# LRMPUT/PUTSLAM

Hardware: AMD Instinct MI355X
Metric: frame-pairs/s (match+RANSAC+Kabsch), 640x480 @ 2000 kpts (higher is better)
Workload: dtype f32; 1 GPU; BASELINE configs[2]: TUM fr1/desk-style synthetic sequence, 500 frames = 499 frame pairs per step per GPU, 2000 kpts/frame, 256-bit descriptors, Hamming BF + cross-check -> depth filter -> H=4096 3-pt Umeyama hypotheses (fixed) scored with errorVersion 1 -> refit; inputs resident in HBM; kpts=2000, hypotheses=4096, world_size=1, force_dist=False, estimator=fixed, streams=4, join=end, submit=ps_batch_queue_submit: whole batches to the library's chains in turn, matcher_kernel=mfma-fused, score_kernel=fast, hw_queues=4, accepted_pairs=499

## Files before the change

putslam_amd/csrc/ps_matcher_mfma.h:

```cpp
#pragma once

#include "ps_kernels.h"

namespace psdev {

typedef int v4i_t __attribute__((ext_vector_type(4)));
typedef int v8i_t __attribute__((ext_vector_type(8)));
typedef float v16f_t __attribute__((ext_vector_type(16)));

constexpr int kTileRows = 32;
constexpr int kTileU4 = 256;
constexpr int kWavesPerWG = kBlock / 64;

PS_D uint32_t fp4_from_byte(uint32_t x)
{
    x = (x | (x << 12)) & 0x000F000Fu;
    x = (x | (x << 6)) & 0x03030303u;
    x = (x | (x << 3)) & 0x11111111u;
    return (x << 3) | 0x66666666u;
}
PS_D v4i_t fp4_from_dword(uint32_t w)
{
    v4i_t r;
    r.x = (int)fp4_from_byte(w & 0xFFu);
    r.y = (int)fp4_from_byte((w >> 8) & 0xFFu);
    r.z = (int)fp4_from_byte((w >> 16) & 0xFFu);
    r.w = (int)fp4_from_byte(w >> 24);
    return r;
}

PS_D int tile_row(int reg, int h) { return (reg & 3) + 8 * (reg >> 2) + 4 * h; }

__global__ __launch_bounds__(kBlock) void ps_expand_query_fp4(const uint32_t *__restrict__ desc,
                                                              const int32_t *__restrict__ nkpts,
                                                              const int32_t *__restrict__ pairs, int cap, int fstride, int tpf,
                                                              int chunks, uint4 *__restrict__ Xq,
                                                              uint32_t *__restrict__ keysInit)
{
    const int p = (int)(blockIdx.x / (unsigned)chunks), chunk = (int)(blockIdx.x % (unsigned)chunks);
    if (keysInit)
        for (int t = chunk * kBlock + threadIdx.x; t < cap; t += chunks * kBlock) keysInit[(size_t)p * cap + t] = kNoKey;
    const int fq = pairs[2 * p];
    const int nq = nkpts[fq];
    const uint32_t *__restrict__ q32 = desc + (size_t)fq * fstride;
    uint4 *__restrict__ out = Xq + (size_t)p * tpf * kTileU4;
    const int o = threadIdx.x, s = o >> 6, h = (o >> 5) & 1, r = o & 31;
    for (int tile = chunk; tile < tpf; tile += chunks) {
        const int row = tile * kTileRows + r;
        v4i_t e = {0, 0, 0, 0};
        if (row < nq) e = fp4_from_dword(q32[(size_t)row * 8 + 2 * s + h]);
        out[(size_t)tile * kTileU4 + o] = make_uint4((uint32_t)e.x, (uint32_t)e.y, (uint32_t)e.z, (uint32_t)e.w);
    }
}

PS_D v16f_t mfma_fp4(const v4i_t &a, const v4i_t &b, const v16f_t &c)
{
    const v8i_t a8 = __builtin_shufflevector(a, a, 0, 1, 2, 3, -1, -1, -1, -1);
    const v8i_t b8 = __builtin_shufflevector(b, b, 0, 1, 2, 3, -1, -1, -1, -1);
    return __builtin_amdgcn_mfma_scale_f32_32x32x64_f8f6f4(a8, b8, c, 4, 4, 0, 0, 0, 0);
}

PS_D v16f_t mfma_fp4s(const v4i_t &a, const v4i_t &b, const v16f_t &c)
{
    const v8i_t a8 = __builtin_shufflevector(a, a, 0, 1, 2, 3, -1, -1, -1, -1);
    const v8i_t b8 = __builtin_shufflevector(b, b, 0, 1, 2, 3, -1, -1, -1, -1);
    return __builtin_amdgcn_mfma_scale_f32_32x32x64_f8f6f4(a8, b8, c, 4, 4, 0, (int)0x88888888u, 0, (int)0x7F7F7F7Fu);
}

PS_D int fbits(float f) { return __builtin_bit_cast(int, f); }
PS_D int imax3(int a, int b, int c) { return max(max(a, b), c); }
PS_D int max16(const v16f_t &d)
{
    int m = imax3(fbits(d[0]), fbits(d[1]), fbits(d[2]));
    m = imax3(m, fbits(d[3]), fbits(d[4]));
    m = imax3(m, fbits(d[5]), fbits(d[6]));
    m = imax3(m, fbits(d[7]), fbits(d[8]));
    m = imax3(m, fbits(d[9]), fbits(d[10]));
    m = imax3(m, fbits(d[11]), fbits(d[12]));
    m = imax3(m, fbits(d[13]), fbits(d[14]));
    return max(m, fbits(d[15]));
}

constexpr float kMfmaNoRow = -1.0e30f;
constexpr int kMfmaBias = 8223;
constexpr float kMfmaBase = 8388608.0f;

#ifndef PS_MFMA_WAVES
#define PS_MFMA_WAVES 1
#endif
template <int TT>
__global__ __launch_bounds__(kBlock, PS_MFMA_WAVES) void ps_hamming_mfma(const uint32_t *__restrict__ desc,
                                                          const int32_t *__restrict__ nkpts,
                                                          const int32_t *__restrict__ pairs, int cap, int fstride, int tpf,
                                                          int groups, int qsplit, const uint4 *__restrict__ Xq,
                                                          uint32_t *__restrict__ keys)
{
    const unsigned perPair = (unsigned)(groups * qsplit);
    const unsigned L = xcd_remap(blockIdx.x, gridDim.x);
    const int p = (int)(L / perPair);
    const int inner = (int)(L - (unsigned)p * perPair);
    const int g = inner / qsplit, qs = inner - g * qsplit;
    const int fq = pairs[2 * p], ft = pairs[2 * p + 1];
    const int nq = nkpts[fq], nt = nkpts[ft];
    if (g * (kWavesPerWG * TT * kTileRows) >= nt) return;
    const int tid = threadIdx.x, lane = tid & 63, wave = tid >> 6;
    const int r = lane & 31, h = lane >> 5;
    const int tile0 = (g * kWavesPerWG + wave) * TT;
    const int nqTiles = (nq + kTileRows - 1) / kTileRows;
    const int T0 = (int)(((long long)nqTiles * qs) / qsplit), T1 = (int)(((long long)nqTiles * (qs + 1)) / qsplit);

    const uint32_t *__restrict__ t32 = desc + (size_t)ft * fstride;
    v4i_t B[TT][4];
#pragma unroll
    for (int i = 0; i < TT; ++i) {
        int t = (tile0 + i) * kTileRows + r;
        t = t < nt ? t : nt - 1;
#pragma unroll
        for (int s = 0; s < 4; ++s) B[i][s] = fp4_from_dword(t32[(size_t)t * 8 + 2 * s + h]);
    }
    v16f_t C;
#pragma unroll
    for (int reg = 0; reg < 16; ++reg) C[reg] = kMfmaBase + (float)(kMfmaBias - 4096 - tile_row(reg, h));
    int best[TT], bestT[TT];
#pragma unroll
    for (int i = 0; i < TT; ++i) {
        best[i] = 0;
        bestT[i] = 0;
    }

    const uint4 *__restrict__ xq = Xq + (size_t)p * tpf * kTileU4;
    uint4 an[4];
    if (T0 < T1) {
#pragma unroll
        for (int s = 0; s < 4; ++s) an[s] = xq[(size_t)T0 * kTileU4 + s * 64 + lane];
    }
    for (int T = T0; T < T1; ++T) {
        v4i_t A[4];
#pragma unroll
        for (int s = 0; s < 4; ++s) {
            A[s].x = (int)an[s].x; A[s].y = (int)an[s].y; A[s].z = (int)an[s].z; A[s].w = (int)an[s].w;
        }
        if (T + 1 < T1) {
#pragma unroll
            for (int s = 0; s < 4; ++s) an[s] = xq[(size_t)(T + 1) * kTileU4 + s * 64 + lane];
        }
        v16f_t Cin = C;
        if (T * kTileRows + kTileRows > nq) {
#pragma unroll
            for (int reg = 0; reg < 16; ++reg)
                if (T * kTileRows + tile_row(reg, h) >= nq) Cin[reg] = kMfmaNoRow;
        }
#pragma unroll
        for (int i = 0; i < TT; ++i) {
            v16f_t acc = mfma_fp4(A[0], B[i][0], Cin);
            acc = mfma_fp4(A[1], B[i][1], acc);
            acc = mfma_fp4(A[2], B[i][2], acc);
            acc = mfma_fp4(A[3], B[i][3], acc);
            const int m = max16(acc);
            if (m > (best[i] | 31)) {
                best[i] = m;
                bestT[i] = T;
            }
        }
    }
#pragma unroll
    for (int i = 0; i < TT; ++i) {
        const int t = (tile0 + i) * kTileRows + r;
        uint32_t key = kNoKey;
        if (best[i] > 0) {
            const int v = kMfmaBias - (best[i] & 0x7FFFFF);
            key = ((uint32_t)(v >> 5) << 16) | (uint32_t)(bestT[i] * kTileRows + (v & 31));
        }
        const uint32_t other = (uint32_t)__shfl_xor((int)key, 32, 64);
        key = other < key ? other : key;
        if (h == 0 && t < nt) {
            if (qsplit == 1)
                keys[(size_t)p * cap + t] = key;
            else
                atomicMin(&keys[(size_t)p * cap + t], key);
        }
    }
}

constexpr int kFuseChunk = 4;

template <int TT>
__global__ __launch_bounds__(kBlock, PS_MFMA_WAVES) void ps_hamming_mfma_fused(const uint32_t *__restrict__ desc,
                                                                const int32_t *__restrict__ nkpts,
                                                                const int32_t *__restrict__ pairs, int cap, int fstride, int tpf,
                                                                int groups, int qsplit, uint32_t *__restrict__ keys)
{
    __shared__ uint4 s_a[2][kFuseChunk][kTileU4];
    __shared__ uint32_t s_lut[256];
    s_lut[threadIdx.x] = fp4_from_byte(threadIdx.x);
    const unsigned perPair = (unsigned)(groups * qsplit);
    const unsigned L = xcd_remap(blockIdx.x, gridDim.x);
    const int p = (int)(L / perPair);
    const int inner = (int)(L - (unsigned)p * perPair);
    const int g = inner / qsplit, qs = inner - g * qsplit;
    const int fq = pairs[2 * p], ft = pairs[2 * p + 1];
    const int nq = nkpts[fq], nt = nkpts[ft];
    if (g * (kWavesPerWG * TT * kTileRows) >= nt) return;
    const int tid = threadIdx.x, lane = tid & 63, wave = tid >> 6;
    const int r = lane & 31, h = lane >> 5;
    const int tile0 = (g * kWavesPerWG + wave) * TT;
    const int nqTiles = (nq + kTileRows - 1) / kTileRows;
    const int T0 = (int)(((long long)nqTiles * qs) / qsplit), T1 = (int)(((long long)nqTiles * (qs + 1)) / qsplit);

    const uint32_t *__restrict__ t32 = desc + (size_t)ft * fstride;
    v4i_t B[TT][4];
#pragma unroll
    for (int i = 0; i < TT; ++i) {
        int t = (tile0 + i) * kTileRows + r;
        t = t < nt ? t : nt - 1;
#pragma unroll
        for (int s = 0; s < 4; ++s) B[i][s] = fp4_from_dword(t32[(size_t)t * 8 + 2 * s + h]);
    }
    v16f_t C;
#pragma unroll
    for (int reg = 0; reg < 16; ++reg) C[reg] = kMfmaBase + (float)((1 << 21) + 31 - tile_row(reg, h));
    int best[TT];
#pragma unroll
    for (int i = 0; i < TT; ++i) best[i] = 0;

    const uint32_t *__restrict__ q32 = desc + (size_t)fq * fstride;
    const int es = tid >> 6, eh = (tid >> 5) & 1, er = tid & 31;
    const int lastT = (nq & (kTileRows - 1)) ? nqTiles - 1 : -1;
    const bool hasPartial = lastT >= T0 && lastT < T1;
    const int Tm = hasPartial ? lastT : T1;
    auto expand_tile = [&](uint4 *dst, int T) {
        const int row = T * kTileRows + er;
        v4i_t e = {0, 0, 0, 0};
        if (row < nq) {
            const uint32_t w = q32[(size_t)row * 8 + 2 * es + eh];
            e.x = (int)s_lut[w & 0xFFu];
            e.y = (int)s_lut[(w >> 8) & 0xFFu];
            e.z = (int)s_lut[(w >> 16) & 0xFFu];
            e.w = (int)s_lut[w >> 24];
        }
        dst[tid] = make_uint4((uint32_t)e.x, (uint32_t)e.y, (uint32_t)e.z, (uint32_t)e.w);
    };
    auto expand_chunk = [&](int buf, int Tc) {
#pragma unroll
        for (int j = 0; j < kFuseChunk; ++j)
            if (Tc + j < Tm) expand_tile(s_a[buf][j], Tc + j);
    };
    auto tile_body = [&](int T, const uint4 *__restrict__ tile, const v16f_t &Cin) {
        v4i_t A[4];
#pragma unroll
        for (int s = 0; s < 4; ++s) {
            const uint4 a = tile[s * 64 + lane];
            A[s].x = (int)a.x; A[s].y = (int)a.y; A[s].z = (int)a.z; A[s].w = (int)a.w;
        }
        const int cT = 16352 - 32 * T;
#pragma unroll
        for (int i = 0; i < TT; ++i) {
            v16f_t acc = mfma_fp4s(A[0], B[i][0], Cin);
            acc = mfma_fp4s(A[1], B[i][1], acc);
            acc = mfma_fp4s(A[2], B[i][2], acc);
            acc = mfma_fp4s(A[3], B[i][3], acc);
            best[i] = max(best[i], max16(acc) + cT);
        }
    };
    __syncthreads();
    if (T0 < Tm) expand_chunk(0, T0);
    __syncthreads();
    int c = 0;
    for (int Tc = T0; Tc < Tm; Tc += kFuseChunk, ++c) {
        if (Tc + kFuseChunk < Tm) expand_chunk((c + 1) & 1, Tc + kFuseChunk);
#pragma unroll 1
        for (int j = 0; j < kFuseChunk; ++j) {
            if (Tc + j >= Tm) break;
            tile_body(Tc + j, s_a[c & 1][j], C);
        }
        __syncthreads();
    }
    if (hasPartial) {
        expand_tile(s_a[0][0], lastT);
        __syncthreads();
        v16f_t Cin = C;
#pragma unroll
        for (int reg = 0; reg < 16; ++reg)
            if (lastT * kTileRows + tile_row(reg, h) >= nq) Cin[reg] = kMfmaNoRow;
        tile_body(lastT, s_a[0][0], Cin);
    }
#pragma unroll
    for (int i = 0; i < TT; ++i) {
        const int t = (tile0 + i) * kTileRows + r;
        uint32_t key = kNoKey;
        if (best[i] > 0) {
            const int d = best[i] & 0x7FFFFF;
            key = ((uint32_t)(256 - (d >> 14)) << 16) | (uint32_t)(16383 - (d & 0x3FFF));
        }
        const uint32_t other = (uint32_t)__shfl_xor((int)key, 32, 64);
        key = other < key ? other : key;
        if (h == 0 && t < nt) {
            if (qsplit == 1)
                keys[(size_t)p * cap + t] = key;
            else
                atomicMin(&keys[(size_t)p * cap + t], key);
        }
    }
}

}
```

Baseline: 591,000 frame-pairs/s.

## Pipeline query loads in registers, replace LUT expansion, use relative max tracking

Swaps the shared-memory byte LUT for a branch-free bitwise fp4 expansion (fp4_word), with static_asserts checking the bit mapping. Query descriptor words are now prefetched into registers one chunk ahead and expanded into the double-buffered shared tile, so global load latency overlaps with MFMA work. Also replaces the per-tile offset add plus max16 with imax3 chains over the float bits and a running relative offset that is rebased once at the end. This lowers ALU and LDS work in the inner loop, at the cost of more complex tail handling and a changed bit-level encoding of the best-match accumulator.

After: 610,100 frame-pairs/s (median of 6 runs). +3.2%, better.

```diff
diff --git a/putslam_amd/csrc/ps_matcher_mfma.h b/putslam_amd/csrc/ps_matcher_mfma.h
--- a/putslam_amd/csrc/ps_matcher_mfma.h
+++ b/putslam_amd/csrc/ps_matcher_mfma.h
@@ -12,20 +12,45 @@
 constexpr int kTileU4 = 256;
 constexpr int kWavesPerWG = kBlock / 64;
 
-PS_D uint32_t fp4_from_byte(uint32_t x)
-{
-    x = (x | (x << 12)) & 0x000F000Fu;
-    x = (x | (x << 6)) & 0x03030303u;
-    x = (x | (x << 3)) & 0x11111111u;
-    return (x << 3) | 0x66666666u;
-}
+PS_HD constexpr uint32_t fp4_word(uint32_t w, int j, uint32_t sign = 0x88888888u, uint32_t fill = 0x66666666u)
+{
+    return (sign & (w << (3 - j))) | (~sign & fill);
+}
+constexpr bool fp4_word_checks(uint32_t w)
+{
+    for (int j = 0; j < 4; ++j) {
+        const uint32_t o = fp4_word(w, j);
+        if ((o & 0x77777777u) != 0x66666666u) return false;
+        for (int i = 0; i < 8; ++i)
+            if (((o >> (4 * i + 3)) & 1u) != ((w >> (4 * i + j)) & 1u)) return false;
+    }
+    return true;
+}
+constexpr bool fp4_single_bits_check()
+{
+    for (int b = 0; b < 32; ++b) {
+        int hits = 0;
+        for (int j = 0; j < 4; ++j)
+            for (int i = 0; i < 8; ++i)
+                if ((fp4_word(1u << b, j) >> (4 * i + 3)) & 1u) hits += (4 * i + j == b) ? 1 : 100;
+        if (hits != 1 || !fp4_word_checks(1u << b) || !fp4_word_checks(~(1u << b))) return false;
+    }
+    return true;
+}
+static_assert(fp4_single_bits_check(), "every descriptor bit is the sign of exactly one nibble");
+static_assert(fp4_word_checks(0u) && fp4_word_checks(0xFFFFFFFFu) && fp4_word_checks(0x80000001u) &&
+                  fp4_word_checks(0xDEADBEEFu) && fp4_word_checks(0x01234567u) && fp4_word_checks(0xA5A5C3C3u) &&
+                  fp4_word_checks(0x0F0F00FFu) && fp4_word_checks(0x13579BDFu),
+              "fp4_word: sign of nibble i of dword j = bit 4 i + j, magnitude 0b110");
+static_assert(fp4_word(0u, 0) == 0x66666666u && fp4_word(0xFFFFFFFFu, 2) == 0xEEEEEEEEu && fp4_word(0x10u, 0) == 0x000000E0u + 0x66666606u,
+              "fp4_word: 0 -> +4.0, 1 -> -4.0");
 PS_D v4i_t fp4_from_dword(uint32_t w)
 {
     v4i_t r;
-    r.x = (int)fp4_from_byte(w & 0xFFu);
-    r.y = (int)fp4_from_byte((w >> 8) & 0xFFu);
-    r.z = (int)fp4_from_byte((w >> 16) & 0xFFu);
-    r.w = (int)fp4_from_byte(w >> 24);
+    r.x = (int)fp4_word(w, 0);
+    r.y = (int)fp4_word(w, 1);
+    r.z = (int)fp4_word(w, 2);
+    r.w = (int)fp4_word(w, 3);
     return r;
 }
 
@@ -191,8 +216,6 @@
                                                                 int groups, int qsplit, uint32_t *__restrict__ keys)
 {
     __shared__ uint4 s_a[2][kFuseChunk][kTileU4];
-    __shared__ uint32_t s_lut[256];
-    s_lut[threadIdx.x] = fp4_from_byte(threadIdx.x);
     const unsigned perPair = (unsigned)(groups * qsplit);
     const unsigned L = xcd_remap(blockIdx.x, gridDim.x);
     const int p = (int)(L / perPair);
@@ -219,77 +242,92 @@
     v16f_t C;
 #pragma unroll
     for (int reg = 0; reg < 16; ++reg) C[reg] = kMfmaBase + (float)((1 << 21) + 31 - tile_row(reg, h));
-    int best[TT];
-#pragma unroll
-    for (int i = 0; i < TT; ++i) best[i] = 0;
+    int rel[TT];
+#pragma unroll
+    for (int i = 0; i < TT; ++i) rel[i] = 0;
 
     const uint32_t *__restrict__ q32 = desc + (size_t)fq * fstride;
     const int es = tid >> 6, eh = (tid >> 5) & 1, er = tid & 31;
     const int lastT = (nq & (kTileRows - 1)) ? nqTiles - 1 : -1;
     const bool hasPartial = lastT >= T0 && lastT < T1;
     const int Tm = hasPartial ? lastT : T1;
-    auto expand_tile = [&](uint4 *dst, int T) {
-        const int row = T * kTileRows + er;
-        v4i_t e = {0, 0, 0, 0};
-        if (row < nq) {
-            const uint32_t w = q32[(size_t)row * 8 + 2 * es + eh];
-            e.x = (int)s_lut[w & 0xFFu];
-            e.y = (int)s_lut[(w >> 8) & 0xFFu];
-            e.z = (int)s_lut[(w >> 16) & 0xFFu];
-            e.w = (int)s_lut[w >> 24];
-        }
-        dst[tid] = make_uint4((uint32_t)e.x, (uint32_t)e.y, (uint32_t)e.z, (uint32_t)e.w);
+    const int nFull = (Tm - T0) / kFuseChunk;
+    const int rem = (Tm - T0) - nFull * kFuseChunk;
+    const int nTail = rem + (hasPartial ? 1 : 0);
+    const int nChunks = nFull + (nTail > 0 ? 1 : 0);
+    const uint32_t *__restrict__ qp = q32 + ((size_t)T0 * kTileRows + er) * 8 + 2 * es + eh;
+    auto load_chunk = [&](int k, uint32_t (&W)[kFuseChunk]) {
+        if (k < nFull) {
+#pragma unroll
+            for (int j = 0; j < kFuseChunk; ++j) W[j] = qp[j * (kTileRows * 8)];
+            qp += kFuseChunk * kTileRows * 8;
+        } else {
+#pragma unroll
+            for (int j = 0; j < kFuseChunk; ++j) {
+                W[j] = 0;
+                if (j < nTail && (T0 + nFull * kFuseChunk + j) * kTileRows + er < nq) W[j] = qp[j * (kTileRows * 8)];
+            }
+        }
     };
-    auto expand_chunk = [&](int buf, int Tc) {
+    uint32_t kSign = 0x88888888u, kFill = 0x66666666u;
+    asm volatile("" : "+s"(kSign), "+v"(kFill));
+    auto expand_chunk = [&](int buf, const uint32_t (&W)[kFuseChunk]) {
 #pragma unroll
         for (int j = 0; j < kFuseChunk; ++j)
-            if (Tc + j < Tm) expand_tile(s_a[buf][j], Tc + j);
+            s_a[buf][j][tid] = make_uint4(fp4_word(W[j], 0, kSign, kFill), fp4_word(W[j], 1, kSign, kFill),
+                                          fp4_word(W[j], 2, kSign, kFill), fp4_word(W[j], 3, kSign, kFill));
     };
-    auto tile_body = [&](int T, const uint4 *__restrict__ tile, const v16f_t &Cin) {
+    auto tile_body = [&](const uint4 *__restrict__ tile, const v16f_t &Cin) {
         v4i_t A[4];
 #pragma unroll
         for (int s = 0; s < 4; ++s) {
             const uint4 a = tile[s * 64 + lane];
             A[s].x = (int)a.x; A[s].y = (int)a.y; A[s].z = (int)a.z; A[s].w = (int)a.w;
         }
-        const int cT = 16352 - 32 * T;
 #pragma unroll
         for (int i = 0; i < TT; ++i) {
             v16f_t acc = mfma_fp4s(A[0], B[i][0], Cin);
             acc = mfma_fp4s(A[1], B[i][1], acc);
             acc = mfma_fp4s(A[2], B[i][2], acc);
             acc = mfma_fp4s(A[3], B[i][3], acc);
-            best[i] = max(best[i], max16(acc) + cT);
+            int m = imax3(rel[i], fbits(acc[0]), fbits(acc[1]));
+#pragma unroll
+            for (int e = 2; e < 16; e += 2) m = imax3(m, fbits(acc[e]), fbits(acc[e + 1]));
+            rel[i] = m + kTileRows;
         }
     };
+    uint32_t W[kFuseChunk] = {0, 0, 0, 0};
+    if (nChunks > 0) {
+        load_chunk(0, W);
+        expand_chunk(0, W);
+    }
+    if (nChunks > 1) load_chunk(1, W);
     __syncthreads();
-    if (T0 < Tm) expand_chunk(0, T0);
-    __syncthreads();
-    int c = 0;
-    for (int Tc = T0; Tc < Tm; Tc += kFuseChunk, ++c) {
-        if (Tc + kFuseChunk < Tm) expand_chunk((c + 1) & 1, Tc + kFuseChunk);
+    for (int k = 0; k < nFull; ++k) {
+        expand_chunk((k + 1) & 1, W);
+        if (k + 2 < nChunks) load_chunk(k + 2, W);
 #pragma unroll 1
-        for (int j = 0; j < kFuseChunk; ++j) {
-            if (Tc + j >= Tm) break;
-            tile_body(Tc + j, s_a[c & 1][j], C);
-        }
+        for (int j = 0; j < kFuseChunk; ++j) tile_body(s_a[k & 1][j], C);
         __syncthreads();
     }
-    if (hasPartial) {
-        expand_tile(s_a[0][0], lastT);
-        __syncthreads();
-        v16f_t Cin = C;
-#pragma unroll
-        for (int reg = 0; reg < 16; ++reg)
-            if (lastT * kTileRows + tile_row(reg, h) >= nq) Cin[reg] = kMfmaNoRow;
-        tile_body(lastT, s_a[0][0], Cin);
-    }
+    if (nTail > 0) {
+#pragma unroll 1
+        for (int j = 0; j < rem; ++j) tile_body(s_a[nFull & 1][j], C);
+        if (hasPartial) {
+            v16f_t Cin = C;
+#pragma unroll
+            for (int reg = 0; reg < 16; ++reg)
+                if (lastT * kTileRows + tile_row(reg, h) >= nq) Cin[reg] = kMfmaNoRow;
+            tile_body(s_a[nFull & 1][rem], Cin);
+        }
+    }
+    const int cEnd = 16352 - kTileRows * T1;
 #pragma unroll
     for (int i = 0; i < TT; ++i) {
         const int t = (tile0 + i) * kTileRows + r;
         uint32_t key = kNoKey;
-        if (best[i] > 0) {
-            const int d = best[i] & 0x7FFFFF;
+        if (rel[i] >= 0x4B000000) {
+            const int d = (rel[i] + cEnd) & 0x7FFFFF;
             key = ((uint32_t)(256 - (d >> 14)) << 16) | (uint32_t)(16383 - (d & 0x3FFF));
         }
         const uint32_t other = (uint32_t)__shfl_xor((int)key, 32, 64);
```
